# rland93/rrtplanner

Measured on AMD Instinct MI355X. Metric: RRT* nodes-expanded/s on 1024x1024 Perlin grid; achieved HBM GB/s, higher is better.
Workload: dtype int16x2 coordinates / u32 squared distances / f64 costs

## Files before the change

rrtplanner_amd/csrc/rrt_block.h:

```cpp
#pragma once

#include "rrt_kernels.h"

namespace rrtdev {

constexpr int BS = 16;

constexpr int TEAM_MAX = 64;
#ifndef RRT_PIPE_LAG
#define RRT_PIPE_LAG 2
#endif
#ifndef RRT_PIPE_LAG_SMALL
#define RRT_PIPE_LAG_SMALL 1
#endif
#ifndef RRT_PIPE_LAG_INF
#define RRT_PIPE_LAG_INF 2
#endif
#ifndef RRT_NPMAX
#define RRT_NPMAX 2
#endif
constexpr int NPMAX = RRT_NPMAX;
#ifndef RRT_PL_MAX
#define RRT_PL_MAX 12
#endif
// ... 52 lines not shown
}

__device__ __forceinline__ uint32_t uni32(uint32_t v) { return (uint32_t)__builtin_amdgcn_readfirstlane((int)v); }
__device__ __forceinline__ int unis32(int v) { return __builtin_amdgcn_readfirstlane(v); }
__device__ __forceinline__ u64 uni64(u64 v) { return ((u64)uni32((uint32_t)(v >> 32)) << 32) | uni32((uint32_t)v); }
__device__ __forceinline__ double unif64(double v) { return __longlong_as_double((long long)uni64((u64)__double_as_longlong(v))); }

__device__ __forceinline__ bool team_wait_all(gu32 *flags, int first, int count, uint32_t target, gu32 *fail, int lane) {
    const u64 t0 = wall_clock64();
    for (;;) {
        const bool mine = lane < count ? __hip_atomic_load(flags + 32 * (first + lane), RRT_RLX_AGENT) >= target : true;
        if (__all(mine)) return true;
        if (__hip_atomic_load(fail, RRT_RLX_AGENT) != 0u) return false;
        if (wall_clock64() - t0 > TEAM_TIMEOUT_TICKS) {
            __hip_atomic_store(fail, 1u, RRT_RLX_AGENT);
            return false;
        }
        __builtin_amdgcn_s_sleep(2);
    }
}

__device__ __forceinline__ bool team_wait(gu32 *word, uint32_t target, gu32 *fail) {
    const u64 t0 = wall_clock64();
    for (;;) {
        if (__hip_atomic_load(word, RRT_RLX_AGENT) >= target) return true;
        if (__hip_atomic_load(fail, RRT_RLX_AGENT) != 0u) return false;
        if (wall_clock64() - t0 > TEAM_TIMEOUT_TICKS) {
            __hip_atomic_store(fail, 1u, RRT_RLX_AGENT);
            return false;
        }
        __builtin_amdgcn_s_sleep(4);
    }
}

__device__ __forceinline__ double sqrt_u24(uint32_t d2) {
    const double x = (double)d2;
    double y = __builtin_amdgcn_rsq(x);
    double g = x * y, h = 0.5 * y;
    double r = __builtin_fma(-h, g, 0.5);
    g = __builtin_fma(g, r, g);
    h = __builtin_fma(h, r, h);
    double d = __builtin_fma(-g, g, x);
    g = __builtin_fma(d, h, g);
    d = __builtin_fma(-g, g, x);
    g = __builtin_fma(d, h, g);
    return d2 == 0 ? 0.0 : g;
}

__device__ __forceinline__ uint32_t key16(uint32_t node_s, uint32_t q_s, uint32_t tag) {
    uint32_t d, r;
    asm("v_pk_sub_i16 %0, %1, %2" : "=v"(d) : "v"(node_s), "s"(q_s));
    asm("v_dot2_i32_i16 %0, %1, %1, %2" : "=v"(r) : "v"(d), "s"(tag));
    return r;
}

struct BRec {
    uint32_t d2s, vs;
    uint32_t los_s;
    uint32_t flags;
    double Vs;
    double cbest;
    uint32_t vbest;
    uint32_t pstat;
    uint32_t nnear;
    float amin;
    double pc;
    u64 nnmask;
    u64 rmask;
    u64 dupmask;
    u64 pnn[NPMAX], pr[NPMAX], pdup[NPMAX];
    u64 plist[PL_WORDS];
};
static_assert(sizeof(BRec) == 8 * BREC_WORDS, "BRec size");
union BRecWords {
    BRec r;
    u64 w[BREC_WORDS];
};

struct BlkState {
    int32_t i, j, nsoln, vbest_soln, pad0, pad1;
    double cmin_soln, c_ell;
};

template <int BSM>
__device__ __forceinline__ void block_scan_step(u32x4 quad, const uint32_t (&xs16)[BSM], uint32_t (&best)[BSM], uint32_t tag0) {
    const uint32_t n0 = quad.x << 4, n1 = quad.y << 4, n2 = quad.z << 4, n3 = quad.w << 4;
#pragma unroll
    for (int k = 0; k < BSM; ++k) {
        const uint32_t k0 = key16(n0, xs16[k], tag0), k1 = key16(n1, xs16[k], tag0 + 1), k2 = key16(n2, xs16[k], tag0 + 2),
                       k3 = key16(n3, xs16[k], tag0 + 3);
        best[k] = min(min(best[k], k0), min(min(k1, k2), k3));
    }
}

struct GSlot {
    double c1, c2;
    uint32_t i1, i2;
    uint32_t hits, nlist;
    uint32_t nn_d2, nn_idx;
    uint32_t pad[2];
    uint32_t x1, x2;
    uint32_t nn_xy, nn_vlo, nn_vhi;
};
struct GCtl {
    double lbc;
    uint32_t lbi, consume;
    double bound;
};

union BlkWords {
    BlkState b;
    u64 w[5];
};

struct ParRound {
    u64 acc_opt, aprev[NPMAX];
    uint32_t list[NWAVE];
    uint32_t accs[64];
    uint32_t count;
    int32_t jp0[NPMAX];
};

template <bool PIPE, bool INF, int BSM>
struct PipeShape {
    static constexpr int LAG = PIPE ? (INF ? RRT_PIPE_LAG_INF : (BSM >= 16 ? RRT_PIPE_LAG_SMALL : RRT_PIPE_LAG)) : 0;
    static_assert(LAG <= NPMAX, "a record carries masks for NPMAX blocks in flight");
    static constexpr int NP = LAG > 0 ? LAG : 1;
    static constexpr int NSLOT = PIPE ? LAG + 1 : 1;
};

template <int G, int BSM, bool PIPE, bool INF>
struct BlockLds {
    static constexpr int SB = BSM * G, NP = PipeShape<PIPE, INF, BSM>::NP;
    alignas(16) u32x2 nnx[(BSM <= BS ? BSM : 1) * NWAVE];
    alignas(16) BRec brec[PIPE ? 2 : 1][SB];
    uint32_t xq_next[PIPE ? 2 : 1][PIPE ? 64 : 1];
    uint32_t pre_state[2];
    alignas(16) BSlot bslots[2 * NWAVE];
    alignas(16) BlkState blk;
    alignas(16) unsigned long long statred[SB * 5];
    uint32_t xq_lds[SB];
    double newcost[SB];
    alignas(16) ParRound par;
    uint32_t xqp_lds[PIPE ? NP : 1][PIPE ? 64 : 1];
    double prevcost[PIPE ? NP : 1][PIPE ? 64 : 1];
    uint32_t help_n[NWAVE], help_x[NWAVE];
    uint32_t help_any;
    uint32_t tick;
    uint32_t slots[BSM >= 16 ? NWAVE : 1][64];
    alignas(16) GSlot gslot[NWAVE];
    alignas(16) GCtl gctl[BSM];
    alignas(8) uint16_t plist[(PIPE && BSM < 16) ? BSM : 1][PL_MAX];
    uint32_t oq_cnt[(PIPE && BSM < 16) ? BSM : 1], oq_ovf;
    uint32_t qhist[16], qstage2;
#ifdef RRT_STAMPS
    unsigned long long dbg[16];
#endif
};

constexpr int ROLE_ALL = 0, ROLE_COMMIT = 1, ROLE_WORK = 2;


template <int G, int BSM, bool PIPE, bool INF, int ROLE, int CW = NWAVE>
__device__ __forceinline__ void rrt_block_body(BatchView bv, BlockLds<G, BSM, PIPE, INF> &L) {
    static_assert(CW == NWAVE || ROLE == ROLE_COMMIT, "only a committer runs with fewer waves");
    constexpr int NTG = CW * 64;
    static_assert(G >= 1 && G <= TEAM_MAX && BSM >= 1 && BSM * G <= 64, "team size");
    constexpr bool WIDE = BSM > BS;
    static_assert(!PIPE || G > 1, "a pipeline needs a team");
    static_assert(PIPE == (ROLE != ROLE_ALL), "roles are the halves of a pipelined team");
    constexpr int LAG = PipeShape<PIPE, INF, BSM>::LAG, NP = PipeShape<PIPE, INF, BSM>::NP, NSLOT = PipeShape<PIPE, INF, BSM>::NSLOT;
    constexpr int SB = BSM * G;
#ifndef RRT_CG16
#define RRT_CG16 2
#endif
    constexpr int CG = (BSM >= 16) ? (ROLE == ROLE_COMMIT ? 2 : RRT_CG16) : 1;
#ifndef RRT_BLOCK_SCATTER
#define RRT_BLOCK_SCATTER 1
#endif
    constexpr bool SCATTER = RRT_BLOCK_SCATTER && BSM >= 16;
    extern __shared__ __attribute__((aligned(16))) unsigned char smem[];
    auto &nnx = L.nnx;
    auto &brec = L.brec;
    auto &xq_next = L.xq_next;
    auto &pre_state = L.pre_state;
    auto &bslots = L.bslots;
    auto &blk = L.blk;
    auto &statred = L.statred;
    auto &xq_lds = L.xq_lds;
    auto &newcost = L.newcost;
    auto &par = L.par;
    auto &xqp_lds = L.xqp_lds;
    auto &prevcost = L.prevcost;
    auto &gslot = L.gslot;
    auto &gctl = L.gctl;
    constexpr int WPS = BSM >= 16 ? 1 : NWAVE / BSM;
    constexpr bool FASTL = PIPE && WPS > 1;
    const int t = (int)threadIdx.x, lane = t & 63, wave = t >> 6;
    int q = (int)blockIdx.x, g_ = 0;
    if (G > 1) {
        q = (int)blockIdx.x % bv.team_qpad;
        g_ = (int)blockIdx.x / bv.team_qpad + bv.member0;
        if (q >= bv.Q) return;
        if (bv.team_fault && g_ == 1) return;
    }
    const int g = ROLE == ROLE_COMMIT ? 0 : g_;
    if (ROLE == ROLE_WORK) __builtin_assume(g > 0);
    const bool worker = !PIPE || ROLE == ROLE_WORK;
    const int wg = PIPE ? (ROLE == ROLE_COMMIT ? 0 : g - 1) : g;
    QDesc *D = bv.desc + q;
    if (D->status != ST_RUNNING) return;
    unsigned char *tb = (G > 1) ? bv.team + (size_t)q * TEAM_BYTES : nullptr;
    gu32 *const t_arrive = (gu32 *)(tb + TEAM_OFF_ARRIVE), *const t_go = (gu32 *)(tb + TEAM_OFF_GO), *const t_fail = (gu32 *)(tb + TEAM_OFF_FAIL);
    gu64 *const t_state = (gu64 *)(tb + TEAM_OFF_STATE), *const t_rec = (gu64 *)(tb + TEAM_OFF_REC);
    uint32_t epoch = 0;
    int pre_i = -1, pre_j = 0;
    constexpr int BSA = WIDE ? 1 : BSM;
    uint32_t pre_xv = 0, pre_best[BSA];
#pragma unroll
    for (int k = 0; k < BSA; ++k) pre_best[k] = NONE;
    bool team_failed = false;
    u64 A_prev[NP];
    int jp0[NP];
#pragma unroll
    for (int p2 = 0; p2 < NP; ++p2) {
        A_prev[p2] = 0;
        jp0[p2] = 0;
    }

    const int n = D->n, alg = D->alg;
    const bool star = alg >= 1, informed = INF && alg == 2;
    const uint32_t *samples = bv.samples + (size_t)q * bv.n_cap;
    uint32_t *nodes_g = bv.nodes + (size_t)q * bv.node_stride;
    const u32x4 *nodes_g4 = reinterpret_cast<const u32x4 *>(nodes_g);
    double *vcost = bv.vcost + (size_t)q * bv.node_stride;
    int32_t *parent = bv.parent + (size_t)q * bv.node_stride;
    uint32_t *bitmap = bv.bitmap + (size_t)q * bv.bitmap_words;
    uint2 *spill = bv.spill + (size_t)q * bv.spill_stride;
    const double *ub = bv.unitball ? bv.unitball + (size_t)q * 2 * bv.n_cap : nullptr;
    const bool logs = bv.nearest_log != nullptr;
    const uint8_t *og = bv.og;
    const int W = bv.W, H = bv.H;
    const int lds_chunks = bv.lds_chunks;
    const int lds_nodes = lds_chunks * CHUNK;
    const uint32_t r2 = D->r2_rewire, goal_d2 = D->goal_d2;
    const uint32_t xs = pack_xy(D->xs[0], D->xs[1]), xg = pack_xy(D->xg[0], D->xg[1]);
    const int ub_offset = D->ub_offset, ub_count = D->ub_count;
    const int cshift = D->cell_shift, ncy = D->ncy, ccap = D->cell_cap, ncells = D->ncx * D->ncy;
    u32x4 *cellrec = reinterpret_cast<u32x4 *>(bv.cellrec) + (size_t)q * (size_t)bv.rec_stride;
    uint32_t *cellcnt_g = bv.cellcnt + (size_t)q * (size_t)MAX_CELLS;
    const bool cells_on = star || BSM >= 16;
    const uint32_t r2h = star ? r2 : (cells_on ? (uint32_t)((2 << cshift) * (2 << cshift)) : 0u);
    int rad = 0;
    if (r2h > 0) {
        rad = (r2h >= (1u << 23)) ? 4096 : (int)sqrtf((float)(r2h - 1));
        while (rad > 0 && (uint32_t)(rad * rad) > r2h - 1) --rad;
        while ((uint32_t)((rad + 1) * (rad + 1)) <= r2h - 1) ++rad;
    }

    RRT_LDS uint32_t *nodes_lds = (RRT_LDS uint32_t *)smem;
    const RRT_LDS u32x4 *nodes_lds4 = (const RRT_LDS u32x4 *)smem;
    RRT_LDS uint32_t *cellcnt = (RRT_LDS uint32_t *)(smem + (size_t)lds_chunks * CHUNK * sizeof(uint32_t));

    int i = D->i, j = D->j;
    int nsoln = D->nsoln, vbest_soln = D->vbest_soln;
    double cmin_soln = D->cmin_soln;
    int i_switch = D->i_switch;
    int status = ST_RUNNING;
#ifdef RRT_STAMPS
    unsigned long long cyc[6] = {D->cyc[0], D->cyc[1], D->cyc[2], D->cyc[3], D->cyc[4], D->cyc[5]};
    unsigned long long tstamp = __builtin_amdgcn_s_memtime();
    unsigned long long wcyc_acc = 0, wcyc_los = 0;
    auto &dbg = L.dbg;
    if (t < 16) dbg[t] = 0;
    unsigned long long dbgt = __builtin_amdgcn_s_memtime();
#ifdef RRT_STAMPS_LIGHT
#define DBGT(k)                                                      \
    do {                                                             \
        if (((RRT_STAMPS_LIGHT) >> (k)) & 1) {                       \
            unsigned long long now_ = __builtin_amdgcn_s_memtime();  \
            if (t == 0) dbg[k] += now_ - dbgt;                       \
            dbgt = now_;                                             \
        }                                                            \
    } while (0)
#else
#define DBGT(k)                                                  \
    do {                                                         \
        unsigned long long now_ = __builtin_amdgcn_s_memtime();  \
        if (t == 0) dbg[k] += now_ - dbgt;                       \
        dbgt = now_;                                             \
    } while (0)
#endif
#else
#define DBGT(k) \
    do {        \
    } while (0)
#endif

#if defined(RRT_STAMPS)
#ifndef RRT_TS_BASE
#define RRT_TS_BASE 300
#endif
#define TSMARK(ep, ev)                                                                                          \
    do {                                                                                                        \
        if ((int)(ep) >= RRT_TS_BASE && (int)(ep) < RRT_TS_BASE + 32 && lane == 0) D->ts[((int)(ep) - RRT_TS_BASE) * 16 + (ev)] = wall_clock64(); \
    } while (0)
#else
#define TSMARK(ep, ev) \
    do {               \
    } while (0)
#endif
#if defined(RRT_STAMPS) && defined(RRT_STAMPS_OWNER)
    unsigned long long wst_ = 0;
#define WST0() (wst_ = __builtin_amdgcn_s_memtime())
#define WST(k)                                                     \
    do {                                                           \
        unsigned long long now_ = __builtin_amdgcn_s_memtime();    \
        if (PIPE && g == 1 && t == 0) dbg[k] += now_ - wst_;       \
        wst_ = now_;                                               \
    } while (0)
#else
#define WST0() \
    do {       \
    } while (0)
#define WST(k) \
    do {       \
    } while (0)
#endif
    const double xc0 = ((double)(D->xs[0] + D->xg[0])) / 2.0, xc1 = ((double)(D->xs[1] + D->xg[1])) / 2.0;
    const double d2sg = (double)dist2(xs, xg);
    const double C00 = D->C[0], C01 = D->C[1], C10 = D->C[2], C11 = D->C[3];
    double c_ell = 0.0;
    if (informed && nsoln > 0) c_ell = cmin_soln + sqrt_u24(dist2(xg, nodes_g[vbest_soln]));

    {
        const uint32_t n0 = nodes_g[0];
        for (int k = t; k < lds_nodes; k += NTG) nodes_lds[k] = (k < j) ? nodes_g[k] : n0;
        for (int k = t; k < ncells; k += NTG) cellcnt[k] = cellcnt_g[k];
        if (t < SB * 5) statred[t] = 0;
        if (t < NWAVE) L.help_n[t] = 0;
        if (t == 0) L.help_any = 0;
        if (t < (int)(sizeof(L.oq_cnt) / sizeof(uint32_t))) L.oq_cnt[t] = 0;
        if (t == 0) L.oq_ovf = 0;
        if (t < 16) L.qhist[t] = 0;
        if (t == 0) L.qstage2 = 0;
    }
    __syncthreads();

    constexpr bool COH = G > 1;
    auto node_xy = [&](uint32_t v) -> uint32_t { return ((int)v < lds_nodes) ? nodes_lds[v] : ld_u32<COH>(nodes_g + v); };
    auto cell_of = [&](uint32_t X) -> int { return (ux(X) >> cshift) * ncy + (uy(X) >> cshift); };

#include "rrt_block_nearset.inc"
    const bool grid_nn = WIDE || rad >= 16;
    if (WIDE && rad < 16) {
        if (t == 0 && g_ == 0) D->status = ST_TEAM_FAIL;
        return;
    }
    auto lower_f32 = [](double c) -> float { return __builtin_fmaxf((float)c * (1.0f - 1.0e-6f) - 4.0e-3f, 0.0f); };
    auto finish_parent = [&](uint32_t X, int j0, double bound, Top2 tt, uint32_t nlist, double &pc, uint32_t &pi, uint32_t &ntests, uint32_t &tcells,
                             float &amin, bool defer, uint32_t &open) {
        pc = f64_inf();
        pi = NONE;
        open = 0;
        amin = tt.i1 == NONE ? FINF : lower_f32(tt.c1);
        if (tt.i1 == NONE || !(tt.c1 < bound)) return;
        amin = tt.i2 == NONE ? FINF : lower_f32(tt.c2);
        if (tt.i2 != NONE && !(tt.c2 < bound)) tt.i2 = NONE;
        bool ok1, ok2;
        int cc1, cc2;
        los_wave2(og, H, node_xy(tt.i1), tt.i2 != NONE ? node_xy(tt.i2) : X, tt.i2 != NONE, X, lane, ok1, cc1, ok2, cc2);
        ntests += 1;
        tcells += (uint32_t)cc1;
        if (ok1) {
            pc = tt.c1;
            pi = tt.i1;
            return;
        }
        if (tt.i2 == NONE) return;
        ntests += 1;
        tcells += (uint32_t)cc2;
        if (ok2) {
            pc = tt.c2;
            pi = tt.i2;
            return;
        }
        amin = 0.0f;
        if (nlist > clist_cap) {
            uint32_t nn2 = 0;
            snapshot_parent(X, j0, false, bound, pc, pi, nn2, ntests, tcells, tt.c2, tt.i2 + 1);
            return;
        }
        uint32_t nval = 0;
        if (defer) {
            consume_price(X, bound, tt.c2, tt.i2 + 1, nlist, nval, amin);
            open = nval;
            return;
        }
        consume_list(X, bound, tt.c2, tt.i2 + 1, nlist, pc, pi, nval, amin);
        count_tests(nval, pc, pi, ntests, tcells);
    };
    auto wave_scan_nearest = [&](uint32_t X, int j0, uint32_t &d2s, uint32_t &vs) {
        uint32_t bd = NONE, bi = NONE;
        for (int base = 0; base < j0; base += 256) {
            const int idx0 = base + 4 * lane;
            if (idx0 < j0) {
                u32x4 v;
                if (idx0 < lds_nodes) v = nodes_lds4[idx0 >> 2];
                else v = ld_rec<COH>(nodes_g4 + (idx0 >> 2));
                const uint32_t pv[4] = {v.x, v.y, v.z, v.w};
#pragma unroll
                for (int e = 0; e < 4; ++e) {
                    const uint32_t d = dist2(pv[e], X);
                    if (idx0 + e < j0 && d < bd) {
                        bd = d;
                        bi = (uint32_t)(idx0 + e);
                    }
                }
            }
        }
        wave_min_key_idx(bd, bi);
        d2s = bd;
        vs = bi;
    };

    const uint32_t node0 = xs;
    auto scan_steps = [&](int c0, int c1, int jlim, const uint32_t (&xs16)[BSA], uint32_t (&best)[BSA]) {
        const int nl = c1 < lds_chunks ? c1 : lds_chunks;
        if (c0 < nl) {
            u32x4 cur = nodes_lds4[c0 * TPB + t];
            for (int c = c0; c < nl; ++c) {
                u32x4 nxt = cur;
                if (c + 1 < nl) nxt = nodes_lds4[(c + 1) * TPB + t];
                block_scan_step<BSA>(cur, xs16, best, (uint32_t)c << 2);
                cur = nxt;
            }
        }
        const int g0 = c0 > nl ? c0 : nl;
        if (c1 > g0) {
            u32x4 cur = nodes_g4[g0 * TPB + t];
            for (int c = g0; c < c1; ++c) {
                u32x4 nxt = cur;
                if (c + 1 < c1) nxt = nodes_g4[(c + 1) * TPB + t];
                if (PIPE) {
                    const int base = c * CHUNK + 4 * t;
                    if (base + 0 >= jlim) cur.x = node0;
                    if (base + 1 >= jlim) cur.y = node0;
                    if (base + 2 >= jlim) cur.z = node0;
                    if (base + 3 >= jlim) cur.w = node0;
                }
                block_scan_step<BSA>(cur, xs16, best, (uint32_t)c << 2);
                cur = nxt;
            }
        }
    };

    constexpr int32_t ST_FLAG_RESTART = 1, ST_FLAG_STOP = 2;
    const bool pipe_inf = PIPE && informed;
    int nprev = 0;
    int void_turns = 0;
    bool prefetched = false;
    bool prefetched_smp = false;
    int bsel = 0;
    auto publish_state = [&](uint32_t ep, int32_t flags) {
        if (lane == 0) {
            BlkWords u;
            u.b.i = i;
            u.b.j = j;
            u.b.nsoln = nsoln;
            u.b.vbest_soln = vbest_soln;
            u.b.pad0 = 0;
            u.b.pad1 = flags;
            u.b.cmin_soln = cmin_soln;
            u.b.c_ell = c_ell;
#pragma unroll
            for (int w = 0; w < 5; ++w) __hip_atomic_store(t_state + (size_t)(ep % NSLOT) * 8 + w, u.w[w], RRT_RLX_AGENT);
        }
        asm volatile("s_waitcnt vmcnt(0)" ::: "memory");
        if (lane == 0) __hip_atomic_store(t_go, ep, RRT_RLX_AGENT);
        if (!grid_nn) __builtin_amdgcn_fence(__ATOMIC_ACQUIRE, "agent");
    };
    while ((pipe_inf && g > 0) || i < n) {
        const int i0 = i, j0 = j;
        int nb = (n - i0) < SB ? (n - i0) : SB;
        const bool ell = informed && nsoln > 0;
        bool void_blk = false;
        if (nb <= 0) {
            nb = 0;
            void_blk = true;
        }
        if (ell) {
            if (i_switch == n) i_switch = i0;
// ... 272 lines not shown
```

rrtplanner_amd/csrc/rrt_block_commit.inc:

```

        BRec r;
        r.d2s = r.vs = r.los_s = r.flags = r.vbest = r.pstat = r.nnear = 0;
        r.amin = 0.0f;
        r.nnmask = r.rmask = r.dupmask = 0;
#pragma unroll
        for (int p2 = 0; p2 < NPMAX; ++p2) r.pnn[p2] = r.pr[p2] = r.pdup[p2] = 0;
        r.Vs = r.cbest = r.pc = 0.0;
        const u64 lbit = 1ull << lane;
        const u64 ltmask = lbit - 1ull;
        bool acc0 = false, goalhit = false, remote_ok = true;
        u64 harm = 0, acc_exact = 0, fin = 0, fin_acc = 0;
        u64 popt = 0, inter = 0, known = 0, aknown = 0;
        bool rounds_on = false;
        bool pbad = false;
        constexpr bool FASTC = PIPE && BSM < 16;
        uint32_t psurv = 0, nent = 0;
        bool lists = false;
        auto cheaper_through = [&](double nc, uint32_t d2, double cb) -> bool {
            const float f = (float)nc + __builtin_amdgcn_sqrtf((float)d2), cf = (float)cb;
            if (f * (1.0f - 1.0e-6f) - 4.0e-3f >= cf * (1.0f + 1.0e-6f) + 4.0e-3f) return false;
            if (f * (1.0f + 1.0e-6f) + 4.0e-3f < cf * (1.0f - 1.0e-6f) - 4.0e-3f) return true;
            return nc + sqrt_u24(d2) < cb;
        };
        auto harmful = [&](int kk) -> bool { return cheaper_through(newcost[kk], dist2(xq_lds[kk], xv), r.cbest); };
// ... 86 lines not shown
                    }
                }
                u64 rm = rk.rmask & acc_k;
                u64 rmp[NP], rmany = rm;
                nnear += (uint32_t)__builtin_popcountll(rm);
#pragma unroll
                for (int p2 = 0; p2 < NP; ++p2) {
                    rmp[p2] = PIPE ? (rk.pr[p2] & ap[p2]) : 0ull;
                    rmany |= rmp[p2];
                    nnear += (uint32_t)__builtin_popcountll(rmp[p2]);
                }
                while (rmany) {
                    double cn = f64_inf();
                    uint32_t ci = NONE;
                    if (rm & lbit) {
                        const double c = newcost[lane] + sqrt_u24(dk);
                        if (c < cnear) {
                            cn = c;
                            ci = 0x80000000u + (uint32_t)NP * 64u + (uint32_t)lane;
                        }
                    }
#pragma unroll
                    for (int p2 = 0; p2 < NP; ++p2) {
                        if (PIPE && (rmp[p2] & lbit)) {
                            const double c = prevcost[p2][lane] + sqrt_u24(dkp[p2]);
                            const uint32_t ref = 0x80000000u + (uint32_t)(NP - 1 - p2) * 64u + (uint32_t)lane;
                            if (c < cnear && key_lt(c, ref, cn, ci)) {
                                cn = c;
                                ci = ref;
                            }
                        }
                    }
                    wave_min_f64_idx(cn, ci);
                    if (ci == NONE || !key_lt(cn, ci, pc, pi)) break;
                    const uint32_t kk = ci & 63u;
                    const int set = (int)((ci - 0x80000000u) >> 6);
                    uint32_t axy = (uint32_t)__builtin_amdgcn_readlane((int)xo, (int)kk);
#pragma unroll
                    for (int p2 = 0; p2 < NP; ++p2)
                        if (set == NP - 1 - p2) axy = (uint32_t)__builtin_amdgcn_readlane((int)xop[p2], (int)kk);
                    int cc = 0;
                    const bool ok = los_wave(og, H, axy, Xk, lane, cc);
                    ntests += 1;
                    tcells += (uint32_t)cc;
                    if (ok) {
                        pc = cn;
                        pi = ci;
                        break;
                    }
                    if (set == NP) rm &= ~(1ull << kk);
#pragma unroll
                    for (int p2 = 0; p2 < NP; ++p2)
                        if (set == NP - 1 - p2) rmp[p2] &= ~(1ull << kk);
                    rmany = rm;
#pragma unroll
                    for (int p2 = 0; p2 < NP; ++p2) rmany |= rmp[p2];
                }
                if (pi != NONE) {
                    vbest = pi;
                    cbest = pc;
                }
            }
            if (lane == 0) {
                BRec &f = brec[bsel][k];
                f.vs = vn;
                f.los_s = cells;
                f.cbest = cbest;
                f.vbest = vbest;
                f.pstat = (ntests << 20) | (tcells & 0xfffffu);
                f.nnear = nnear;
                f.flags = rk.flags | 2u;
                newcost[k] = cbest;
            }
#if defined(RRT_STAMPS) && !defined(RRT_STAMPS_LIGHT)
            if (t == 0) {
                dbg[rs_redo ? 10 : 12] += __builtin_amdgcn_s_memtime() - rs0;
                dbg[rs_redo ? 11 : 5] += 1;
            }
#endif
        };

        auto fast_settle = [&](u64 hm, uint32_t ps, uint32_t ne, u64 rmask_own) {
            if constexpr (FASTC) {
                BRec &f = brec[bsel][lane];
                const uint32_t own0 = ne - (uint32_t)__builtin_popcountll(rmask_own);
                uint32_t cm = ps;
                while (hm) {
                    const int kk = __builtin_ctzll(hm);
                    hm &= hm - 1;
                    cm |= 1u << (own0 + (uint32_t)__builtin_popcountll(rmask_own & lowmask64(kk)));
                }
                auto entry_of = [&](uint32_t pe) -> uint32_t { return (uint32_t)(f.plist[pe >> 2] >> (16u * (pe & 3u))) & 0xffffu; };
                auto entry_cost = [&](uint32_t e16) -> double {
                    const int kk = (int)(e16 & 63u), set = (int)((e16 >> 6) & 3u);
                    if (set == NP) return newcost[kk] + sqrt_u24(dist2(xq_lds[kk], xv));
                    return prevcost[NP - 1 - set][kk] + sqrt_u24(dist2(xqp_lds[NP - 1 - set][kk], xv));
                };
                double bc = f64_inf();
                uint32_t bref = NONE, bcells = 0, nblocked = 0;
                for (uint32_t m = cm; m != 0; m &= m - 1) {
                    const uint32_t e16 = entry_of((uint32_t)__builtin_ctz(m));
                    if ((e16 >> 15) == 0u) {
                        nblocked += 1;
                        continue;
                    }
                    const double c = entry_cost(e16);
                    const uint32_t ref = 0x80000000u + (e16 & 0xffu);
                    if (key_lt(c, ref, bc, bref)) {
                        bc = c;
                        bref = ref;
                        bcells = (e16 >> 8) & 127u;
                    }
                }
                uint32_t nt = bref != NONE ? 1u : 0u, tc = bcells;
                if (nblocked != 0) {
                    for (uint32_t m = cm; m != 0; m &= m - 1) {
                        const uint32_t e16 = entry_of((uint32_t)__builtin_ctz(m));
                        if ((e16 >> 15) != 0u) continue;
                        if (bref == NONE || key_lt(entry_cost(e16), 0x80000000u + (e16 & 0xffu), bc, bref)) {
                            nt += 1;
                            tc += (e16 >> 8) & 127u;
                        }
                    }
                }
                const uint32_t ps0 = f.pstat;
                f.pstat = (((ps0 >> 20) + nt) << 20) | (((ps0 & 0xfffffu) + tc) & 0xfffffu);
                if (bref != NONE) {
                    f.cbest = bc;
                    f.vbest = bref;
                    newcost[lane] = bc;
                }
            }
        };

        auto fetch_records = [&](uint32_t ep, int half) {
            constexpr int NCH = SB * BREC_WORDS * 8 / 16, NIT = (NCH + 63) / 64;
            static_assert(NCH * 16 == SB * BREC_WORDS * 8, "whole chunks");
            const unsigned char *src = tb + TEAM_OFF_REC + (size_t)(ep % NSLOT) * 64 * BREC_WORDS * 8;
            u32x4 v[NIT];
#pragma unroll
            for (int it = 0; it < NIT; ++it) {
                const int c = it * 64 + lane;
                v[it] = ld_b128_agent(src + 16 * (c < NCH ? c : NCH - 1));
            }
            fence_b128s(v);
            RRT_LDS u32x4 *dst = (RRT_LDS u32x4 *)&brec[half][0];
#pragma unroll
            for (int it = 0; it < NIT; ++it) {
                const int c = it * 64 + lane;
                if (c < NCH) dst[c] = v[it];
            }
        };

        if (wave == 0) {
            if (G > 1) {
                DBGT(7);
                if (PIPE && prefetched) {
                    remote_ok = uni32(pre_state[bsel]) == 1u;
                } else {
                    remote_ok = team_wait_all(t_arrive, 1, PIPE ? G : G - 1, epoch, t_fail, lane);
                    if (PIPE) {
                        if (remote_ok) fetch_records(epoch, bsel);
                    } else if (remote_ok && lane >= BSM && lane < nb) {
                        const gu64 *src = t_rec + (size_t)(epoch % NSLOT) * 64 * BREC_WORDS + (size_t)lane * BREC_WORDS;
                        BRecWords u;
#pragma unroll
                        for (int w = 0; w < BREC_WORDS; ++w) u.w[w] = __hip_atomic_load(src + w, RRT_RLX_AGENT);
                        brec[bsel][lane] = u.r;
                    }
                }
            }
            DBGT(7);
            if (ROLE == ROLE_COMMIT) TSMARK(epoch, 11);
            if (!remote_ok) {
                if (lane == 0) blk.pad0 = 1;
            } else {
                if (lane < nb) r = brec[bsel][lane];
                acc0 = lane < nb && (r.los_s >> 31) != 0 && (r.flags & 1u) == 0;
                goalhit = informed && lane < nb && dist2(xv, xg) < goal_d2;
                if (lane < nb) newcost[lane] = r.cbest;
                if (PIPE && epoch == 1) {
#pragma unroll
                    for (int p2 = 0; p2 < NP; ++p2) jp0[p2] = j0;
                }
                if constexpr (FASTC) {
                    nent = (r.flags >> 8) & 0xffu;
                    lists = lane < nb && nent <= (uint32_t)PL_MAX;
                }
                if (lane < nb && acc0) {
                    u64 rm = r.rmask;
                    while (rm) {
                        const int kk = __builtin_ctzll(rm);
                        rm &= rm - 1;
                        if (harmful(kk)) harm |= 1ull << kk;
                    }
                }
                if (PIPE && lane < nb) {
#pragma unroll
                    for (int p2 = 0; p2 < NP; ++p2) {
                        pbad = pbad || ((r.pnn[p2] | r.pdup[p2]) & A_prev[p2]) != 0;
                        if (acc0) {
                            u64 rm = r.pr[p2] & A_prev[p2];
                            uint32_t pbase = 0;
#pragma unroll
                            for (int p3 = NP - 1; p3 > p2; --p3) pbase += (uint32_t)__builtin_popcountll(r.pr[p3]);
                            while (rm) {
                                const int kk = __builtin_ctzll(rm);
                                rm &= rm - 1;
                                if (cheaper_through(prevcost[p2][kk], dist2(xqp_lds[p2][kk], xv), r.cbest)) {
                                    if (FASTC && lists) psurv |= 1u << (pbase + (uint32_t)__builtin_popcountll(r.pr[p2] & lowmask64(kk)));
                                    else pbad = true;
                                }
                            }
                        }
                    }
                }
                if (PIPE) {
                    popt = __ballot(acc0);
                    inter = (r.nnmask | r.dupmask | r.rmask) & ltmask;
                    const bool slow0 = lane < nb && (((r.nnmask | r.dupmask | harm) & popt & ltmask) != 0 || pbad || psurv != 0);
                    u64 taint = __ballot(slow0);
                    for (int it = 0; it < 6; ++it) {
                        const u64 t2 = taint | __ballot(lane < nb && (inter & taint) != 0);
                        if (t2 == taint) break;
                        taint = t2;
                        if (it == 5) taint = ~0ull;
                    }
                    known = ~taint;
                    aknown = popt & ~taint;
                    rounds_on = j0 + __builtin_popcountll(popt) < n;
                }
            }
        }
        DBGT(1);
        if (PIPE) {
            u64 lastmask = 0;
            for (;;) {
                DBGT(2);
                if (wave == 0) {
                    uint32_t cnt = 0;
                    u64 newacc = 0;
                    if (lastmask != 0) {
                        newacc = __ballot(((lastmask >> lane) & 1ull) != 0 && par.accs[lane] != 0u);
                        fin |= lastmask;
                        fin_acc |= newacc;
                        known |= lastmask;
                        aknown |= newacc;
                    }
                    if (remote_ok && rounds_on && (~known & lowmask64(nb)) != 0) {
                        if (newacc != 0) {
                            u64 rm = r.rmask & newacc;
                            if (lane < nb && acc0) {
                                while (rm) {
                                    const int kk = __builtin_ctzll(rm);
                                    rm &= rm - 1;
                                    harm = (harm & ~(1ull << kk)) | (harmful(kk) ? (1ull << kk) : 0ull);
                                }
                            }
                        }
                        u64 L0 = 0;
                        for (;;) {
                            const bool ready = lane < nb && (known & lbit) == 0 && (inter & ~known) == 0;
                            const bool hd = (harm & aknown & ltmask) != 0;
                            const bool sd = ((r.nnmask | r.dupmask) & aknown & ltmask) != 0 || pbad || (goalhit && acc0) || (hd && !(FASTC && lists));
                            const bool fd = FASTC && !sd && (hd || psurv != 0);
                            const u64 cb = __ballot(ready && !sd && !fd);
                            const u64 fb = FASTC ? __ballot(ready && fd) : 0ull;
                            if (cb == 0 && fb == 0) {
                                L0 = __ballot(ready && sd && !goalhit);
                                break;
                            }
                            known |= cb;
                            aknown |= cb & popt;
                            if constexpr (FASTC) {
                                if (fb != 0) {
                                    if (ready && fd) fast_settle(harm & aknown & ltmask, psurv, nent, r.rmask);
                                    fin |= fb;
                                    fin_acc |= fb;
                                    known |= fb;
                                    aknown |= fb;
#ifdef RRT_STAMPS
                                    if (t == 0) dbg[13] += (unsigned long long)__builtin_popcountll(fb) << 32;
#endif
                                    u64 rm = r.rmask & fb;
                                    if (lane < nb && acc0 && (known & lbit) == 0) {
                                        while (rm) {
                                            const int kk = __builtin_ctzll(rm);
                                            rm &= rm - 1;
                                            harm = (harm & ~(1ull << kk)) | (harmful(kk) ? (1ull << kk) : 0ull);
                                        }
                                    }
                                }
                            }
                        }
                        const uint32_t place = (uint32_t)__builtin_popcountll(L0 & ltmask);
                        const bool listed = ((L0 >> lane) & 1ull) != 0 && place < (uint32_t)CW;
                        if (listed) par.list[place] = (uint32_t)lane;
                        lastmask = __ballot(listed);
                        cnt = (uint32_t)__builtin_popcountll(lastmask);
#ifdef RRT_STAMPS
                        if (t == 0) dbg[6] += cnt;
                        if (t == 0 && cnt != 0) dbg[13] += 1;
#endif
                        if (lane == 0 && cnt != 0) {
                            par.acc_opt = aknown;
#pragma unroll
                            for (int p2 = 0; p2 < NP; ++p2) {
                                par.aprev[p2] = A_prev[p2];
                                par.jp0[p2] = jp0[p2];
                            }
                        }
                    }
                    if (lane == 0) par.count = cnt;
                }
                DBGT(8);
                __syncthreads();
                const uint32_t cnt = uni32(par.count);
                if (cnt == 0) break;
                if ((uint32_t)wave < cnt) {
                    const int k = (int)uni32(par.list[wave]);
                    bool acc;
                    double cb;
                    u64 ap[NP];
                    int jp[NP];
#pragma unroll
                    for (int p2 = 0; p2 < NP; ++p2) {
                        ap[p2] = uni64(par.aprev[p2]);
                        jp[p2] = unis32(par.jp0[p2]);
                    }
                    resolve_sample(k, uni64(par.acc_opt) & lowmask64(k), ap, jp, false, acc, cb);
                    if (lane == 0) par.accs[k] = acc ? 1u : 0u;
                }
                __syncthreads();
            }
        }
        DBGT(2);
        const bool pre_next = PIPE && (!informed || LAG >= 2) && i0 + nb < n;
        const bool pre_smp = pre_next && !informed;
        if (PIPE && wave == CW - 1 && pre_next) {
#ifdef RRT_STAMPS
            const unsigned long long pf0 = __builtin_amdgcn_s_memtime();
#endif
            TSMARK(epoch, 2);
#if defined(RRT_STAMPS) && !defined(RRT_STAMPS_LIGHT)
            bool ok = true;
            {
                const u64 t0w = wall_clock64();
                u64 lastmiss = 0;
                for (;;) {
                    const bool mine = lane < G ? __hip_atomic_load(t_arrive + 32 * (1 + lane), RRT_RLX_AGENT) >= epoch + 1 : true;
                    const u64 miss = __ballot(!mine);
                    if (miss == 0) break;
                    if (!mine) D->dbg2[lane] += 1;
                    lastmiss = miss;
                    if (__hip_atomic_load(t_fail, RRT_RLX_AGENT) != 0u || wall_clock64() - t0w > TEAM_TIMEOUT_TICKS) {
                        ok = false;
                        break;
                    }
                    __builtin_amdgcn_s_sleep(2);
                }
                if (lastmiss != 0 && (lastmiss & (lastmiss - 1)) == 0 && ((lastmiss >> lane) & 1ull)) D->dbg2[64 + lane] += 1;
            }
#else
            const bool ok = team_wait_all(t_arrive, 1, G, epoch + 1, t_fail, lane);
#endif
#ifdef RRT_STAMPS
            const unsigned long long pf1 = __builtin_amdgcn_s_memtime();
#endif
            TSMARK(epoch, 3);
            if (ok) fetch_records(epoch + 1, bsel ^ 1);
            TSMARK(epoch, 4);
            if (lane == 0) pre_state[bsel ^ 1] = ok ? 1u : 2u;
#ifdef RRT_STAMPS
            if (lane == 0) dbg[14] += ((__builtin_amdgcn_s_memtime() - pf0) & 0xffffffffull) | ((pf1 - pf0) << 32);
#endif
        }
        if (PIPE && wave == CW - 2 && pre_smp) {
            const int in = i0 + nb;
            const int nbn = (n - in) < SB ? (n - in) : SB;
            if (lane < nbn) xq_next[bsel ^ 1][lane] = at32(samples, (uint32_t)(in + lane));
        }
        if (wave == 0 && remote_ok) {
            int cur = 0;
            bool cut = false;
            const double c_ell0 = c_ell;
            const bool myacc0 = (fin & lbit) ? (fin_acc & lbit) != 0 : acc0;
            while (cur < nb && !cut) {
                const u64 pend = __ballot(myacc0 && lane >= cur);
                const u64 Aopt = acc_exact | (pend & ltmask);
                const bool slow = lane >= cur && lane < nb && (fin & lbit) == 0 &&
                                  (((r.nnmask | r.dupmask | harm) & Aopt) != 0 || pbad || psurv != 0 || (goalhit && acc0));
                const unsigned long long bad = __ballot(slow);
                const int k0 = bad ? (int)__builtin_ctzll(bad) : nb;
                acc_exact |= pend & lowmask64(k0) & ~lowmask64(cur);
                cur = k0;
                if (cur >= nb) break;
                {
                    const int k = cur;
                    const int jk = j0 + __builtin_popcountll(acc_exact);
                    const uint32_t Xk = (uint32_t)__builtin_amdgcn_readlane((int)xv, k);
                    bool acc;
                    double cbest;
                    resolve_sample(k, acc_exact, A_prev, jp0, true, acc, cbest);

                    if (acc) {
                        if (informed && dist2(Xk, xg) < goal_d2) {
                            const bool first = nsoln == 0;
                            nsoln++;
                            if (cbest < cmin_soln) {
                                cmin_soln = cbest;
                                vbest_soln = jk;
                                c_ell = cmin_soln + sqrt_u24(dist2(xg, Xk));
                                cut = true;
                            }
                            if (first) cut = true;
                        }
                        acc_exact |= 1ull << k;
                        const bool redo = lane > k && lane < nb && acc0 && ((r.rmask >> k) & 1ull) != 0;
                        if (__ballot(redo) != 0 && redo) harm = (harm & ~(1ull << k)) | (harmful(k) ? (1ull << k) : 0ull);
                    }
                    cur = k + 1;
                }
            }
            DBGT(3);
            {
                if (j0 + __builtin_popcountll(acc_exact) > n) acc_exact &= ~(1ull << (63 - __builtin_clzll(acc_exact)));
                const bool inr = lane < cur;
                const BRec f0 = brec[bsel][lane];
                BRec f = f0;
                auto node_of = [&](uint32_t v) -> uint32_t {
                    if (v == NONE || (v & 0x80000000u) == 0) return v;
                    const int kk = (int)(v & 63u);
                    const int set = (int)((v - 0x80000000u) >> 6);
                    uint32_t node = (uint32_t)j0 + (uint32_t)__builtin_popcountll(acc_exact & lowmask64(kk));
#pragma unroll
                    for (int p2 = 0; p2 < NP; ++p2)
                        if (set == NP - 1 - p2) node = (uint32_t)jp0[p2] + (uint32_t)__builtin_popcountll(A_prev[p2] & lowmask64(kk));
                    return node;
                };
                f.vs = node_of(f.vs);
                f.vbest = node_of(f.vbest);
                const bool myacc = inr && ((acc_exact >> lane) & 1ull) != 0;
                const int jmine = j0 + __builtin_popcountll(acc_exact & ltmask);
                if (inr) {
                    statred[lane * 5 + 0] += (unsigned long long)jmine;
                    statred[lane * 5 + 1] += (unsigned long long)(f.los_s & 0x7fffffffu);
                    if (logs) {
                        const size_t o = (size_t)q * bv.n_cap + i0 + lane;
                        bv.nearest_log[o] = (int32_t)f.vs;
                        bv.accept_log[o] = (uint8_t)myacc;
                        bv.cbest_log[o] = ell ? c_ell0 : __longlong_as_double(0x7ff8000000000000ll);
                        bv.j_log[o] = jmine;
                    }
                }
                if (myacc) {
                    if (star) {
                        uint32_t nprevnear = 0;
#pragma unroll
                        for (int p2 = 0; p2 < NP; ++p2) nprevnear += PIPE ? (uint32_t)__builtin_popcountll(f.pr[p2] & A_prev[p2]) : 0u;
                        statred[lane * 5 + 2] += (f.flags & 2u) ? f.nnear
                                                       : f.nnear + (uint32_t)__builtin_popcountll(f.rmask & acc_exact & ltmask) + nprevnear;
                        statred[lane * 5 + 4] += f.pstat >> 20;
                        statred[lane * 5 + 3] += f.pstat & 0xfffffu;
                    }
                    const uint32_t cellbit = (uint32_t)ux(xv) * (uint32_t)H + (uint32_t)uy(xv);
                    if (jmine < lds_nodes) nodes_lds[jmine] = xv;
                    const unsigned long long cb = (unsigned long long)__double_as_longlong(f.cbest);
                    if (G > 1) {
                        __hip_atomic_store((gu32 *)&at32(nodes_g, (uint32_t)jmine), xv, RRT_RLX_AGENT);
                        __hip_atomic_store((gu64 *)&at32(vcost, (uint32_t)jmine), (u64)cb, RRT_RLX_AGENT);
                        __hip_atomic_store((gu32 *)&at32(parent, (uint32_t)jmine), f.vbest, RRT_RLX_AGENT);
                    } else {
                        at32(nodes_g, (uint32_t)jmine) = xv;
                        at32(vcost, (uint32_t)jmine) = f.cbest;
                        at32(parent, (uint32_t)jmine) = (int32_t)f.vbest;
                    }
                    atomicOr(&at32(bitmap, cellbit >> 5), 1u << (cellbit & 31));
                    if (cells_on) {
                        const int c = cell_of(xv);
                        const uint32_t slot = __hip_atomic_fetch_add(&cellcnt[c], 1u, __ATOMIC_RELAXED, __HIP_MEMORY_SCOPE_WORKGROUP);
                        u32x4 rc = {xv, (uint32_t)jmine, (uint32_t)cb, (uint32_t)(cb >> 32)};
                        if (G > 1) {
                            gu64 *dst = (gu64 *)&at32(cellrec, (uint32_t)c * (uint32_t)ccap + slot);
                            __hip_atomic_store(dst, ((u64)jmine << 32) | xv, RRT_RLX_AGENT);
                            __hip_atomic_store(dst + 1, (u64)cb, RRT_RLX_AGENT);
                        } else {
                            at32(cellrec, (uint32_t)c * (uint32_t)ccap + slot) = rc;
                        }
                    }
                }
                j = j0 + __builtin_popcountll(acc_exact);
                if (PIPE) {
#pragma unroll
                    for (int p2 = NP - 1; p2 > 0; --p2) {
                        xqp_lds[p2][lane] = xqp_lds[p2 - 1][lane];
                        prevcost[p2][lane] = prevcost[p2 - 1][lane];
                        A_prev[p2] = A_prev[p2 - 1];
                        jp0[p2] = jp0[p2 - 1];
                    }
                    xqp_lds[0][lane] = xv;
                    prevcost[0][lane] = f.cbest;
                    A_prev[0] = acc_exact;
                    jp0[0] = j0;
                }
            }
            i = i0 + cur;
            if (lane == 0) {
                BlkState b;
                b.i = i;
                b.j = j;
                b.nsoln = nsoln;
                b.vbest_soln = vbest_soln;
                b.pad0 = 0;
                b.pad1 = (PIPE && cut) ? ST_FLAG_RESTART : 0;
                b.cmin_soln = cmin_soln;
                b.c_ell = c_ell;
                blk = b;
            }
            DBGT(9);
            if (G > 1) publish_state(epoch, (PIPE && cut) ? ST_FLAG_RESTART : 0);
            if (ROLE == ROLE_COMMIT) TSMARK(epoch, 1);
            DBGT(4);
        }
```

Baseline: 6.280 million.

## Defer commit store pass to a second wave and bound prefetch wait

For the pipelined non-informed committer running with fewer waves, the per-round store pass (node, cost, parent, bitmap and cell-record writes plus state publish) is split into a lambda. Wave 0 no longer runs it inline: it saves the accept masks and indices to LDS, and wave 1 runs the pass and publishes state at the start of the next round. The prefetch of the next epoch's records now polls team arrival only a bounded number of times, and marks a 'late' state that falls back to a blocking wait later. The aim is to take global stores and publishing off wave 0's critical path and stop it spinning on stragglers. The cost is more LDS state and a publish that happens one step later, which could delay the worker waves.

```diff
diff --git a/rrtplanner_amd/csrc/rrt_block.h b/rrtplanner_amd/csrc/rrt_block.h
--- a/rrtplanner_amd/csrc/rrt_block.h
+++ b/rrtplanner_amd/csrc/rrt_block.h
@@ -228,6 +228,12 @@
     alignas(16) GCtl gctl[BSM];
     alignas(8) uint16_t plist[(PIPE && BSM < 16) ? BSM : 1][PL_MAX];
     uint32_t oq_cnt[(PIPE && BSM < 16) ? BSM : 1], oq_ovf;
+    struct Defer {
+        unsigned long long acc, aprev[NPMAX];
+        int jp0[NPMAX];
+        int cur, j0, i0, bsel;
+        uint32_t epoch, pending;
+    } defer;
     uint32_t qhist[16], qstage2;
 #ifdef RRT_STAMPS
     unsigned long long dbg[16];
@@ -414,6 +420,7 @@
         for (int k = t; k < lds_nodes; k += NTG) nodes_lds[k] = (k < j) ? nodes_g[k] : n0;
         for (int k = t; k < ncells; k += NTG) cellcnt[k] = cellcnt_g[k];
         if (t < SB * 5) statred[t] = 0;
+        if (t == 0) L.defer.pending = 0;
         if (t < NWAVE) L.help_n[t] = 0;
         if (t == 0) L.help_any = 0;
         if (t < (int)(sizeof(L.oq_cnt) / sizeof(uint32_t))) L.oq_cnt[t] = 0;
diff --git a/rrtplanner_amd/csrc/rrt_block_commit.inc b/rrtplanner_amd/csrc/rrt_block_commit.inc
--- a/rrtplanner_amd/csrc/rrt_block_commit.inc
+++ b/rrtplanner_amd/csrc/rrt_block_commit.inc
@@ -262,11 +262,96 @@
             }
         };
 
+        auto store_pass = [&](u64 accx, int curx, int j0x, int i0x, int bselx, const u64 (&apx)[NP], const int (&jpx)[NP], uint32_t xvx, double cell_log) {
+            const bool inr = lane < curx;
+            BRec f = brec[bselx][lane];
+            auto node_of = [&](uint32_t v) -> uint32_t {
+                if (v == NONE || (v & 0x80000000u) == 0) return v;
+                const int kk = (int)(v & 63u);
+                const int set = (int)((v - 0x80000000u) >> 6);
+                uint32_t node = (uint32_t)j0x + (uint32_t)__builtin_popcountll(accx & lowmask64(kk));
+#pragma unroll
+                for (int p2 = 0; p2 < NP; ++p2)
+                    if (set == NP - 1 - p2) node = (uint32_t)jpx[p2] + (uint32_t)__builtin_popcountll(apx[p2] & lowmask64(kk));
+                return node;
+            };
+            f.vs = node_of(f.vs);
+            f.vbest = node_of(f.vbest);
+            const bool myacc = inr && ((accx >> lane) & 1ull) != 0;
+            const int jmine = j0x + __builtin_popcountll(accx & ltmask);
+            if (inr) {
+                statred[lane * 5 + 0] += (unsigned long long)jmine;
+                statred[lane * 5 + 1] += (unsigned long long)(f.los_s & 0x7fffffffu);
+                if (logs) {
+                    const size_t o = (size_t)q * bv.n_cap + i0x + lane;
+                    bv.nearest_log[o] = (int32_t)f.vs;
+                    bv.accept_log[o] = (uint8_t)myacc;
+                    bv.cbest_log[o] = cell_log;
+                    bv.j_log[o] = jmine;
+                }
+            }
+            if (myacc) {
+                if (star) {
+                    uint32_t nprevnear = 0;
+#pragma unroll
+                    for (int p2 = 0; p2 < NP; ++p2) nprevnear += PIPE ? (uint32_t)__builtin_popcountll(f.pr[p2] & apx[p2]) : 0u;
+                    statred[lane * 5 + 2] += (f.flags & 2u) ? f.nnear
+                                                   : f.nnear + (uint32_t)__builtin_popcountll(f.rmask & accx & ltmask) + nprevnear;
+                    statred[lane * 5 + 4] += f.pstat >> 20;
+                    statred[lane * 5 + 3] += f.pstat & 0xfffffu;
+                }
+                const uint32_t cellbit = (uint32_t)ux(xvx) * (uint32_t)H + (uint32_t)uy(xvx);
+                if (jmine < lds_nodes) nodes_lds[jmine] = xvx;
+                const unsigned long long cb = (unsigned long long)__double_as_longlong(f.cbest);
+                if (G > 1) {
+                    __hip_atomic_store((gu32 *)&at32(nodes_g, (uint32_t)jmine), xvx, RRT_RLX_AGENT);
+                    __hip_atomic_store((gu64 *)&at32(vcost, (uint32_t)jmine), (u64)cb, RRT_RLX_AGENT);
+                    __hip_atomic_store((gu32 *)&at32(parent, (uint32_t)jmine), f.vbest, RRT_RLX_AGENT);
+                } else {
+                    at32(nodes_g, (uint32_t)jmine) = xvx;
+                    at32(vcost, (uint32_t)jmine) = f.cbest;
+                    at32(parent, (uint32_t)jmine) = (int32_t)f.vbest;
+                }
+                atomicOr(&at32(bitmap, cellbit >> 5), 1u << (cellbit & 31));
+                if (cells_on) {
+                    const int c = cell_of(xvx);
+                    const uint32_t slot = __hip_atomic_fetch_add(&cellcnt[c], 1u, __ATOMIC_RELAXED, __HIP_MEMORY_SCOPE_WORKGROUP);
+                    u32x4 rc = {xvx, (uint32_t)jmine, (uint32_t)cb, (uint32_t)(cb >> 32)};
+                    if (G > 1) {
+                        gu64 *dst = (gu64 *)&at32(cellrec, (uint32_t)c * (uint32_t)ccap + slot);
+                        __hip_atomic_store(dst, ((u64)jmine << 32) | xvx, RRT_RLX_AGENT);
+                        __hip_atomic_store(dst + 1, (u64)cb, RRT_RLX_AGENT);
+                    } else {
+                        at32(cellrec, (uint32_t)c * (uint32_t)ccap + slot) = rc;
+                    }
+                }
+            }
+        };
+        constexpr bool DEFER = PIPE && !INF && ROLE == ROLE_COMMIT && CW < NWAVE;
+        if constexpr (DEFER) {
+            if (wave == 1 && uni32(L.defer.pending) != 0u) {
+                u64 ap_[NP];
+                int jp_[NP];
+#pragma unroll
+                for (int p2 = 0; p2 < NP; ++p2) {
+                    ap_[p2] = uni64(L.defer.aprev[p2]);
+                    jp_[p2] = unis32(L.defer.jp0[p2]);
+                }
+                store_pass(uni64(L.defer.acc), unis32(L.defer.cur), unis32(L.defer.j0), unis32(L.defer.i0), unis32(L.defer.bsel), ap_, jp_,
+                           xqp_lds[0][lane], __longlong_as_double(0x7ff8000000000000ll));
+                const uint32_t epd = uni32(L.defer.epoch);
+                publish_state(epd, 0);
+                TSMARK(epd, 1);
+                if (lane == 0) L.defer.pending = 0;
+            }
+        }
+
         if (wave == 0) {
             if (G > 1) {
                 DBGT(7);
-                if (PIPE && prefetched) {
-                    remote_ok = uni32(pre_state[bsel]) == 1u;
+                const uint32_t pst = (PIPE && prefetched) ? uni32(pre_state[bsel]) : 3u;
+                if (pst != 3u) {
+                    remote_ok = pst == 1u;
                 } else {
                     remote_ok = team_wait_all(t_arrive, 1, PIPE ? G : G - 1, epoch, t_fail, lane);
                     if (PIPE) {
@@ -452,9 +537,16 @@
             const unsigned long long pf0 = __builtin_amdgcn_s_memtime();
 #endif
             TSMARK(epoch, 2);
+            bool ok = false, late = false;
+            if constexpr (DEFER) {
+                for (int look = 0; look < 3 && !ok; ++look) {
+                    const bool mine = lane < G ? __hip_atomic_load(t_arrive + 32 * (1 + lane), RRT_RLX_AGENT) >= epoch + 1 : true;
+                    ok = __all(mine);
+                }
+                late = !ok;
+            } else {
 #if defined(RRT_STAMPS) && !defined(RRT_STAMPS_LIGHT)
-            bool ok = true;
-            {
+                ok = true;
                 const u64 t0w = wall_clock64();
                 u64 lastmiss = 0;
                 for (;;) {
@@ -470,17 +562,17 @@
                     __builtin_amdgcn_s_sleep(2);
                 }
                 if (lastmiss != 0 && (lastmiss & (lastmiss - 1)) == 0 && ((lastmiss >> lane) & 1ull)) D->dbg2[64 + lane] += 1;
-            }
 #else
-            const bool ok = team_wait_all(t_arrive, 1, G, epoch + 1, t_fail, lane);
-#endif
+                ok = team_wait_all(t_arrive, 1, G, epoch + 1, t_fail, lane);
+#endif
+            }
 #ifdef RRT_STAMPS
             const unsigned long long pf1 = __builtin_amdgcn_s_memtime();
 #endif
             TSMARK(epoch, 3);
             if (ok) fetch_records(epoch + 1, bsel ^ 1);
             TSMARK(epoch, 4);
-            if (lane == 0) pre_state[bsel ^ 1] = ok ? 1u : 2u;
+            if (lane == 0) pre_state[bsel ^ 1] = ok ? 1u : (late ? 3u : 2u);
 #ifdef RRT_STAMPS
             if (lane == 0) dbg[14] += ((__builtin_amdgcn_s_memtime() - pf0) & 0xffffffffull) | ((pf1 - pf0) << 32);
 #endif
@@ -535,72 +627,26 @@
             DBGT(3);
             {
                 if (j0 + __builtin_popcountll(acc_exact) > n) acc_exact &= ~(1ull << (63 - __builtin_clzll(acc_exact)));
-                const bool inr = lane < cur;
-                const BRec f0 = brec[bsel][lane];
-                BRec f = f0;
-                auto node_of = [&](uint32_t v) -> uint32_t {
-                    if (v == NONE || (v & 0x80000000u) == 0) return v;
-                    const int kk = (int)(v & 63u);
-                    const int set = (int)((v - 0x80000000u) >> 6);
-                    uint32_t node = (uint32_t)j0 + (uint32_t)__builtin_popcountll(acc_exact & lowmask64(kk));
-#pragma unroll
-                    for (int p2 = 0; p2 < NP; ++p2)
-                        if (set == NP - 1 - p2) node = (uint32_t)jp0[p2] + (uint32_t)__builtin_popcountll(A_prev[p2] & lowmask64(kk));
-                    return node;
-                };
-                f.vs = node_of(f.vs);
-                f.vbest = node_of(f.vbest);
-                const bool myacc = inr && ((acc_exact >> lane) & 1ull) != 0;
-                const int jmine = j0 + __builtin_popcountll(acc_exact & ltmask);
-                if (inr) {
-                    statred[lane * 5 + 0] += (unsigned long long)jmine;
-                    statred[lane * 5 + 1] += (unsigned long long)(f.los_s & 0x7fffffffu);
-                    if (logs) {
-                        const size_t o = (size_t)q * bv.n_cap + i0 + lane;
-                        bv.nearest_log[o] = (int32_t)f.vs;
-                        bv.accept_log[o] = (uint8_t)myacc;
-                        bv.cbest_log[o] = ell ? c_ell0 : __longlong_as_double(0x7ff8000000000000ll);
-                        bv.j_log[o] = jmine;
-                    }
-                }
-                if (myacc) {
-                    if (star) {
-                        uint32_t nprevnear = 0;
-#pragma unroll
-                        for (int p2 = 0; p2 < NP; ++p2) nprevnear += PIPE ? (uint32_t)__builtin_popcountll(f.pr[p2] & A_prev[p2]) : 0u;
-                        statred[lane * 5 + 2] += (f.flags & 2u) ? f.nnear
-                                                       : f.nnear + (uint32_t)__builtin_popcountll(f.rmask & acc_exact & ltmask) + nprevnear;
-                        statred[lane * 5 + 4] += f.pstat >> 20;
-                        statred[lane * 5 + 3] += f.pstat & 0xfffffu;
-                    }
-                    const uint32_t cellbit = (uint32_t)ux(xv) * (uint32_t)H + (uint32_t)uy(xv);
-                    if (jmine < lds_nodes) nodes_lds[jmine] = xv;
-                    const unsigned long long cb = (unsigned long long)__double_as_longlong(f.cbest);
-                    if (G > 1) {
-                        __hip_atomic_store((gu32 *)&at32(nodes_g, (uint32_t)jmine), xv, RRT_RLX_AGENT);
-                        __hip_atomic_store((gu64 *)&at32(vcost, (uint32_t)jmine), (u64)cb, RRT_RLX_AGENT);
-                        __hip_atomic_store((gu32 *)&at32(parent, (uint32_t)jmine), f.vbest, RRT_RLX_AGENT);
-                    } else {
-                        at32(nodes_g, (uint32_t)jmine) = xv;
-                        at32(vcost, (uint32_t)jmine) = f.cbest;
-                        at32(parent, (uint32_t)jmine) = (int32_t)f.vbest;
-                    }
-                    atomicOr(&at32(bitmap, cellbit >> 5), 1u << (cellbit & 31));
-                    if (cells_on) {
-                        const int c = cell_of(xv);
-                        const uint32_t slot = __hip_atomic_fetch_add(&cellcnt[c], 1u, __ATOMIC_RELAXED, __HIP_MEMORY_SCOPE_WORKGROUP);
-                        u32x4 rc = {xv, (uint32_t)jmine, (uint32_t)cb, (uint32_t)(cb >> 32)};
-                        if (G > 1) {
-                            gu64 *dst = (gu64 *)&at32(cellrec, (uint32_t)c * (uint32_t)ccap + slot);
-                            __hip_atomic_store(dst, ((u64)jmine << 32) | xv, RRT_RLX_AGENT);
-                            __hip_atomic_store(dst + 1, (u64)cb, RRT_RLX_AGENT);
-                        } else {
-                            at32(cellrec, (uint32_t)c * (uint32_t)ccap + slot) = rc;
-                        }
-                    }
+                const bool defer_now = DEFER && i0 + cur < n;
+                if (!defer_now) {
+                    store_pass(acc_exact, cur, j0, i0, bsel, A_prev, jp0, xv, ell ? c_ell0 : __longlong_as_double(0x7ff8000000000000ll));
+                } else if (lane == 0) {
+                    L.defer.acc = acc_exact;
+#pragma unroll
+                    for (int p2 = 0; p2 < NP; ++p2) {
+                        L.defer.aprev[p2] = A_prev[p2];
+                        L.defer.jp0[p2] = jp0[p2];
+                    }
+                    L.defer.cur = cur;
+                    L.defer.j0 = j0;
+                    L.defer.i0 = i0;
+                    L.defer.bsel = bsel;
+                    L.defer.epoch = epoch;
+                    L.defer.pending = 1u;
                 }
                 j = j0 + __builtin_popcountll(acc_exact);
                 if (PIPE) {
+                    const double cfin = brec[bsel][lane].cbest;
 #pragma unroll
                     for (int p2 = NP - 1; p2 > 0; --p2) {
                         xqp_lds[p2][lane] = xqp_lds[p2 - 1][lane];
@@ -609,26 +655,28 @@
                         jp0[p2] = jp0[p2 - 1];
                     }
                     xqp_lds[0][lane] = xv;
-                    prevcost[0][lane] = f.cbest;
+                    prevcost[0][lane] = cfin;
                     A_prev[0] = acc_exact;
                     jp0[0] = j0;
                 }
-            }
-            i = i0 + cur;
-            if (lane == 0) {
-                BlkState b;
-                b.i = i;
-                b.j = j;
-                b.nsoln = nsoln;
-                b.vbest_soln = vbest_soln;
-                b.pad0 = 0;
-                b.pad1 = (PIPE && cut) ? ST_FLAG_RESTART : 0;
-                b.cmin_soln = cmin_soln;
-                b.c_ell = c_ell;
-                blk = b;
-            }
-            DBGT(9);
-            if (G > 1) publish_state(epoch, (PIPE && cut) ? ST_FLAG_RESTART : 0);
-            if (ROLE == ROLE_COMMIT) TSMARK(epoch, 1);
-            DBGT(4);
+                i = i0 + cur;
+                if (lane == 0) {
+                    BlkState b;
+                    b.i = i;
+                    b.j = j;
+                    b.nsoln = nsoln;
+                    b.vbest_soln = vbest_soln;
+                    b.pad0 = 0;
+                    b.pad1 = (PIPE && cut) ? ST_FLAG_RESTART : 0;
+                    b.cmin_soln = cmin_soln;
+                    b.c_ell = c_ell;
+                    blk = b;
+                }
+                DBGT(9);
+                if (!defer_now) {
+                    if (G > 1) publish_state(epoch, (PIPE && cut) ? ST_FLAG_RESTART : 0);
+                    if (ROLE == ROLE_COMMIT) TSMARK(epoch, 1);
+                }
+                DBGT(4);
+            }
         }
```

After: 6.361 million, median of 6. +1.3%, better.
